# a-rtemis99/hpc_suffix_array

Hardware: AMD Instinct MI355X
Metric: suffixes sorted/sec + ms/doubling-round, 1 GiB input at 1/2/4/8 MI355X (higher is better)
Workload: dtype u32

## Files before the change

### hpc_suffix_array_amd/_native.py

```python
from __future__ import annotations

import ctypes
import os
import subprocess

PKG_DIR = os.path.dirname(os.path.abspath(__file__))
LIB_PATH = os.path.join(PKG_DIR, "lib", "libsa_hip.so")
LIB_PATH = os.environ.get("SA_LIB_PATH", LIB_PATH)
CSRC = os.path.join(PKG_DIR, "csrc")

SA_MAX_ROUNDS = 64
KERNEL_KINDS = ["init", "hist_first", "hist_keys", "scan", "scatter_first", "scatter_keys",
                "heads", "heads_scan", "rerank", "seg_count", "seg_scan", "seg_write", "alphabet", "pack",
                "sort_u", "windows", "local_sort", "pivot_keys", "pivot_count", "pivot_write"]
SCHEDULE_PACKED = 0
SCHEDULE_REFERENCE = 1
ROUND1_AUTO = 0
ROUND1_LSD = 1
ROUND1_BUCKETED = 2
SA_K_COUNT = len(KERNEL_KINDS)
FIND_AUTO = 0
FIND_LANE = 1
FIND_WAVE = 2
FIND_LANE_MAX = 3584
# ... 8 lines not shown
               "sa_count_below_u64_device", "sa_select_u8_device",
               "sa_find_device", "sa_find", "sa_find_ex",
               "sa_match_device", "sa_matching_stats_device", "sa_match", "sa_matching_stats",
               "sa_dist_begin", "sa_dist_cuts", "sa_dist_plan_cuts", "sa_dist_reserve", "sa_dist_release", "sa_dist_round1", "sa_dist_req_count", "sa_dist_req_fill",
               "sa_dist_answer", "sa_dist_refine",
               "sa_last_error", "sa_host_syncs", "sa_device_count", "sa_version", "sa_struct_size"]


class SAError(RuntimeError):
    """A libsa_hip entry point returned an error code."""


DEBUG_FLAGS = {"no_cmp": 0x1, "no_pk8": 0x2, "no_pad": 0x4, "pad_overflow": 0x8, "no_fast32": 0x10,
               "no_pivot": 0x20, "perm_always": 0x40, "no_xq": 0x80, "xq_overflow": 0x100,
               "no_tied": 0x200, "no_key1_round": 0x400, "no_eonly": 0x800,
               "eonly": 0x1000, "fast32_small": 0x2000}


def debug_bits(names) -> int:
    bits = 0
    for x in names or ():
        if x not in DEBUG_FLAGS:
            raise ValueError(f"unknown debug flag {x!r} (one of {sorted(DEBUG_FLAGS)})")
        bits |= DEBUG_FLAGS[x]
    return bits


class SaOpts(ctypes.Structure):
    _fields_ = [("profile", ctypes.c_int32), ("schedule", ctypes.c_int32), ("init_chars", ctypes.c_int32),
                ("radix", ctypes.c_int32), ("round1", ctypes.c_int32), ("debug", ctypes.c_uint32),
                ("span_extra", ctypes.c_int32), ("tune", ctypes.c_int32)]
# ... 217 lines not shown
```

### hpc_suffix_array_amd/csrc/sa_bucket.h

```cpp
#pragma once
#include "sa_kernels.h"

namespace sa {

#ifndef SA_BS_BLOCK
#define SA_BS_BLOCK 512
#endif
constexpr int kBsBlock = SA_BS_BLOCK;
#ifndef SA_BS_ITEMS
#define SA_BS_ITEMS 18
#endif
constexpr int kBsItems = SA_BS_ITEMS;
constexpr int kBsCap = kBsBlock * kBsItems;
constexpr uint32_t kWinStride = 1024;
#ifndef SA_BS_WPC
#define SA_BS_WPC 2
#endif
constexpr uint32_t kBsWpc = SA_BS_WPC;
#ifndef SA_BS_GRID
#define SA_BS_GRID (1u << 22)
#endif
constexpr uint32_t kBsGrid = SA_BS_GRID;
constexpr uint64_t kBucketMinN = 1ull << 20;
constexpr uint32_t kLoBits = 8;
// ... 810 lines not shown
    const uint32_t nlist = words[7];
    const uint32_t lane = lane_id();
    for (uint64_t q = (uint64_t)blockIdx.x * kWaves + wave_id(); q < nlist; q += (uint64_t)gridDim.x * kWaves) {
        const uint32_t j = list[q];
        const uint32_t a = ws[j], o = ou[j], c = ou[j + 1] - o, g0 = og[j];
        for (uint32_t k = lane; k < c; k += kWave) {
            const uint32_t x = so.tmp_idx[a + k];
            u_pos[o + k] = so.tmp_pos[a + k];
            u_idx[o + k] = x;
            u_g[o + k] = so.tmp_g[a + k] + g0;
            if (so.tmp_rank) so.rank[rm.slot(x)] = so.tmp_rank[a + k];
        }
    }
}

constexpr int kPcPer = 16;
constexpr int kPcBlock = kBlock * kPcPer;

__device__ __forceinline__ void popc_load(const uint32_t* __restrict__ bits, uint64_t nw, uint64_t b0,
                                          uint32_t (&c)[kPcPer]) {
    if (b0 + kPcPer <= nw) {
#pragma unroll
        for (int q = 0; q < kPcPer / 4; ++q) {
            const uint4 v = reinterpret_cast<const uint4*>(bits + b0)[q];
            c[4 * q] = (uint32_t)__popc(v.x);
            c[4 * q + 1] = (uint32_t)__popc(v.y);
            c[4 * q + 2] = (uint32_t)__popc(v.z);
            c[4 * q + 3] = (uint32_t)__popc(v.w);
        }
    } else {
// ... 1085 lines not shown
```

### hpc_suffix_array_amd/csrc/sa_build.hip

```cpp
#include <hip/hip_runtime.h>

#include <algorithm>
#include <atomic>
#include <chrono>
#include <cstdarg>
#include <cstdio>
#include <cstdlib>
#include <cstring>
#include <mutex>
#include <string>
#include <thread>
#include <vector>

#include "../../include/sa_hip.h"

#ifndef SA_ALPHA_GRID
#define SA_ALPHA_GRID 2048
#endif

#include "sa_bucket.h"
#include "sa_check.h"
#include "sa_kernels.h"
#include "sa_lcp.h"
#include "sa_limits.h"
// ... 18 lines not shown
}

#define SA_HIP(call)                                                                         \
    do {                                                                                     \
        hipError_t e_ = (call);                                                              \
        if (e_ != hipSuccess)                                                                \
            return set_err(SA_E_HIP, "%s failed: %s (%s:%d)", #call, hipGetErrorString(e_),  \
                           __FILE__, __LINE__);                                              \
    } while (0)

static std::atomic<uint64_t> g_host_syncs{0};
static hipError_t host_sync(hipStream_t s) {
    g_host_syncs.fetch_add(1, std::memory_order_relaxed);
    return hipStreamSynchronize(s);
}
static hipError_t host_memcpy(void* dst, const void* src, size_t bytes, hipMemcpyKind kind) {
    g_host_syncs.fetch_add(1, std::memory_order_relaxed);
    return hipMemcpy(dst, src, bytes, kind);
}

#define SA_TRY(...)                      \
    do {                                 \
        const int rc_ = (__VA_ARGS__);   \
        if (rc_) return rc_;             \
    } while (0)

static bool trace_on() {
    static const bool on = std::getenv("SA_TRACE") != nullptr;
    return on;
}
// ... 1 lines not shown
    do {                                                \
        if (trace_on()) {                               \
            std::fprintf(stderr, "[sa] " __VA_ARGS__);  \
            std::fputc('\n', stderr);                   \
        }                                               \
    } while (0)

#ifndef SA_MAX_CHUNKS
#define SA_MAX_CHUNKS 4096
#endif
constexpr uint32_t kMaxChunks = SA_MAX_CHUNKS;
static_assert(kMaxChunks >= 1 && kMaxChunks <= (1u << 20), "chunk scratch sized for at most 2^20 chunks");
constexpr uint64_t kSparseDiv = 8;
constexpr int kEvPool = 256;
constexpr int kRoundEv = SA_MAX_ROUNDS + 1;

static uint64_t align_up(uint64_t x, uint64_t a) { return (x + a - 1) / a * a; }

static uint32_t bit_width(uint64_t x) {
    uint32_t w = 0;
    while (x) { ++w; x >>= 1; }
    return w;
}

static Chunking plan_chunks(uint64_t n) {
    Chunking ch;
    ch.n = n;
    const uint64_t tiles = (n + kTile - 1) / kTile;
    uint64_t tpc = (tiles + kMaxChunks - 1) / kMaxChunks;
    if (tpc == 0) tpc = 1;
// ... 28 lines not shown
    uint32_t* lsd = nullptr;
    uint32_t* lsdx = nullptr;
    uint32_t* segw = nullptr;
    uint64_t* states = nullptr;
    uint32_t epoch = 0;
    int radix = 0;
    int cus = 256;
    uint32_t* member = nullptr;
    uint32_t* hist = nullptr;
    uint32_t* totals = nullptr;
    uint32_t* counts = nullptr;
    uint32_t* words = nullptr;
    uint32_t* alpha = nullptr;
    uint16_t* code = nullptr;
    uint32_t* host_words = nullptr;
    hipEvent_t ev[sa::kEvPool + sa::kRoundEv];
    int ev_ready = 0;
    sa::DistState* dist = nullptr;
    uint32_t dbg = 0;
    int32_t span_extra = 0;
    int32_t tune = 0;
    bool dna = false;
    bool samples_pending = false;
};

namespace sa {

static uint64_t pad_capacity(uint64_t n) { return n + n / 8 + (1ull << 22); }

static uint64_t pad_elems(uint64_t n) {
    const uint64_t m = align_up(std::max<uint64_t>(n, 1), 64);
// ... 144 lines not shown
        if (!on) return;
        hipEventRecord(c->ev[2 * used + 1], s);
        ++used;
    }
    int nr = 0;
    uint64_t mark_bytes[kRoundEv] = {};
    void round_mark() {
        if (nr < kRoundEv) {
            hipEventRecord(c->ev[kEvPool + nr], s);
            uint64_t b = 0;
            if (st)
                for (int k = 0; k < SA_K_COUNT; ++k) b += st->kern_bytes[k];
            mark_bytes[nr] = b;
        }
        ++nr;
    }
    void round_times() {
        const int last = std::min(nr, kRoundEv) - 1;
        if (!st || last < 1) return;
        hipEventSynchronize(c->ev[kEvPool + last]);
        for (int r = 0; r < last && r < st->rounds; ++r) {
            float ms = 0.f;
            hipEventElapsedTime(&ms, c->ev[kEvPool + r], c->ev[kEvPool + r + 1]);
            st->round_ms[r] = ms;
            st->round_bytes[r] = mark_bytes[r + 1] - mark_bytes[r];
        }
    }
    void flush() {
        if (!on || used == 0) return;
        hipEventSynchronize(c->ev[2 * used - 1]);
// ... 626 lines not shown
    const uint64_t base = (uint64_t)sigma + 1;
    const uint32_t kmax = max_chars(base);
    if (req > 0) return std::min<uint32_t>((uint32_t)req, kmax);
    if (sigma <= 1) return kmax;
    const uint32_t kmin = min_chars(sigma, n);
    const uint32_t P = (key_bits(base, kmin) + 7) / 8;
    uint32_t K = kmin;
    while (K + 1 <= kmax && key_bits(base, K + 1) <= 8 * P) ++K;
    return K;
}

constexpr uint64_t kUsAvg = 4;
#ifndef SA_US_TWO_PHASE
#define SA_US_TWO_PHASE 1
#endif
constexpr int kUsFlagWord = 12;

template <class Pos>
static int segments(sa_context* c, const uint64_t* keys, const uint32_t* idx, const Chunking& ch, Pos pos,
                    bool sparse_ok, bool* sparse_out,
                    uint32_t* sa, int uo, hipStream_t s, Timer& tm, sa_stats* st, uint64_t* D, uint64_t* m,
                    uint64_t* G, uint32_t* rank_arr = nullptr, uint64_t rank_off = 0, RankMap rm = RankMap{},
                    uint64_t set_off = 0, uint32_t g_off = 0, uint32_t* gsn = nullptr) {
    if (!rank_arr) rank_arr = c->rank;
    uint32_t* c_h = c->counts;
    uint32_t* c_u = c->counts + kMaxChunks;
    uint32_t* c_uh = c->counts + 2 * kMaxChunks;
    uint32_t* c_l = c->counts + 3 * kMaxChunks;
    tm.begin(SA_K_SEG_COUNT);
    hipLaunchKernelGGL(k_seg_count, dim3(ch.chunks), dim3(kBlock), 0, s, keys, ch, c_h, c_u, c_uh, c_l);
    tm.end();
// ... 286 lines not shown
    if (bucketed && bp.bs.cmp && short_suffix_ties(h_tail, n, tail_n, h_code, sigma, bp.bs.s, bp.bs.R))
        bucketed = plan_bucketed(sigma, n, Kb, r1, c->radix, &bp, 1, 0);
    const bool force_eonly = (c->dbg & SA_DEBUG_EONLY) != 0;
    if (bucketed && bp.bs.cmp == 1 && ((sigma & (sigma - 1)) != 0 || force_eonly) && !(c->dbg & SA_DEBUG_NO_EONLY)) {
        const uint32_t hb = bp.bs.bb - kLoBits;
        BucketPlan b2;
        if ((force_eonly || !plan_pk8(bp, hb, c->dbg, true)) && plan_bucketed(sigma, n, Kb, r1, c->radix, &b2, 1, 2) &&
            (force_eonly || plan_pk8(b2, hb, c->dbg, true)) &&
            !short_suffix_ties(h_tail, n, tail_n, h_code, sigma, b2.bs.s, b2.bs.R, b2.K))
            bp = b2;
    }
    bool fused = false;
    bool r1_pivot = false;
    uint64_t D = 0, m = 0, G = 0;
    uint64_t seg1[3] = {0, 0, 0};
    if (bucketed) {
        bool done = false;
        rc = round1_bucketed(c, d_text, n, d_sa, bp, full_range(bp, n), s, tm, st, &done, &fused, seg1, &ksh1);
        if (rc) return rc;
        bucketed = done;
        if (done) {
            keys1 = c->keys[0];
            P = 2;
            K = bp.K;
        }
    }
    if (!bucketed) {
        const uint32_t bits1 = key_bits(base, K);
        SA_TRACE("packed: sigma=%u K=%u bits=%u", sigma, K, bits1);
        uint64_t top = 1;
        for (uint32_t t = 1; t < K; ++t) top *= base;
        if (c->radix == 0) {
            rc = onesweep_prepare(c, s);
// ... 43 lines not shown
                        bucketed ? 1u : 0u, bp.bs, bucketed ? c->segw + kBstartOff : nullptr, d_sa, ksh1};
    if (st) st->sparse_ranks = sparse ? 1 : 0;
    auto ensure_samples = [&]() -> int {
        if (!c->samples_pending) return SA_OK;
        c->samples_pending = false;
        const uint64_t ns = (n + (1ull << ksh1) - 1) >> ksh1;
        const uint32_t g = (uint32_t)std::max<uint64_t>(1, std::min<uint64_t>((ns + kBlock - 1) / kBlock, 8192));
        tm.begin(SA_K_SORT_U);
        hipLaunchKernelGGL(k_key1_samples, dim3(g), dim3(kBlock), 0, s, d_text, n, (const uint16_t*)c->code, bp.bs,
                           (const uint32_t*)d_sa, ksh1, keys1);
        tm.end();
        SA_HIP(hipGetLastError());
        add_bytes(st, SA_K_SORT_U, 12 * ns);
        return SA_OK;
    };
    tm.round_mark();
    record_round(st, 0.f, D, P, n, K);
    SA_TRACE("  round 1: D=%llu unsorted=%llu groups=%llu", (unsigned long long)D, (unsigned long long)m,
             (unsigned long long)G);

    const uint32_t wr = bit_width(n);
    for (uint64_t h = K; m > 0; h *= 2) {
        if (h >= 2 * n) return set_err(SA_E_INTERNAL, "doubling did not converge (h=%llu)", (unsigned long long)h);
        const uint32_t wg = G > 1 ? bit_width(G - 1) : 0;
        const uint32_t bits = wg + wr;
        if (bits > 64) return set_err(SA_E_INTERNAL, "key of %u bits", bits);
        const Chunking cu = plan_chunks(m);
        const int ui = uo;
        uo ^= 1;
        uint64_t* sorted = nullptr;
        bool segs_done = false;
        uint64_t Du = 0, m2 = 0, G2 = 0;
        uint32_t kb1 = 0;
        if (bucketed && sparse && h == K && !(c->dbg & SA_DEBUG_NO_KEY1_ROUND)) {
            unsigned __int128 dmax = 1;
            for (uint32_t t = 0; t < bp.bs.s; ++t) dmax *= bp.bs.sigma;
            const unsigned __int128 kmax = ((dmax - 1) << bp.bs.rb) | (((unsigned __int128)1 << bp.bs.rb) - 1);
            uint32_t kw = 0;
            for (unsigned __int128 x = kmax + 1; x; x >>= 1) ++kw;
            kb1 = kw;
        }
        const bool key1_round = kb1 > 0 && kb1 + wg <= 64;
        if (c->radix == 0 && G > 0 && m <= kUsAvg * G) {
            if (sparse && !(SA_US_TWO_PHASE && key1_round)) {
                rc = ensure_samples();
                if (rc) return rc;
            }
            SA_HIP(hipMemsetAsync(c->words + kUsFlagWord, 0, 4, s));
            const uint32_t grid = (uint32_t)std::min<uint64_t>((m + kBlock - 1) / kBlock, 8192);
            tm.begin(SA_K_SORT_U);
#if SA_US_TWO_PHASE
            const uint32_t gk = (uint32_t)std::min<uint64_t>((m + kBlock - 1) / kBlock, 65536);
            if (sparse && key1_round)
                hipLaunchKernelGGL(k_usort_keys<SrcUKey1>, dim3(gk), dim3(kBlock), 0, s,
                                   SrcUKey1{c->u_idx[ui], c->u_g[ui], rl, h, kb1}, m, ukb0);
            else if (sparse)
// ... 543 lines not shown
    if (hipDeviceGetAttribute(&c->cus, hipDeviceAttributeMultiprocessorCount, device) != hipSuccess || c->cus <= 0)
        c->cus = 256;
    if (hipMalloc(&c->hist, (size_t)kRadix * kMaxChunks * 4) != hipSuccess ||
        hipMalloc(&c->totals, kRadix * 4) != hipSuccess || hipMalloc(&c->counts, 4 * kMaxChunks * 4) != hipSuccess ||
        hipMalloc(&c->words, 64) != hipSuccess || hipMalloc(&c->alpha, 256 * 4) != hipSuccess ||
        hipMalloc(&c->code, 256 * 2) != hipSuccess ||
        hipMalloc(&c->os, (2 * kMaxPasses * kRadix + kMaxPasses) * 4) != hipSuccess ||
        hipMalloc(&c->lsd, (2 * kMaxPasses * kLsdMaxRadix + kMaxPasses) * 4 + 64) != hipSuccess ||
        hipMalloc(&c->lsdx, kLsdXqWords * 4) != hipSuccess ||
        hipMalloc(&c->segw, (kBstartOff + 2 * kBstartWords) * 4) != hipSuccess ||
        hipHostMalloc(&c->host_words, 16384, hipHostMallocDefault) != hipSuccess) {
        (void)hipGetLastError();
        sa_context_destroy(c);
        return set_err(SA_E_NOMEM, "context allocation failed");
    }
    for (int i = 0; i < kEvPool + kRoundEv; ++i) {
        if (hipEventCreate(&c->ev[i]) != hipSuccess) {
            sa_context_destroy(c);
            return set_err(SA_E_HIP, "hipEventCreate failed");
        }
        c->ev_ready = i + 1;
    }
    if (max_n) {
        int rc = ensure_capacity(c, max_n);
        if (rc) {
            sa_context_destroy(c);
            return rc;
        }
    }
    *out = c;
    return SA_OK;
// ... 588 lines not shown
```

### hpc_suffix_array_amd/csrc/sa_round1.h

```cpp
#pragma once

#ifndef SA_HIST_WPC
#define SA_HIST_WPC 64
#endif
#ifndef SA_REC_STRIPED
#define SA_REC_STRIPED 1
#endif
#ifndef SA_BB_EXTRA
#define SA_BB_EXTRA 0
#endif
#ifndef SA_ITEMS_A
#define SA_ITEMS_A 12
#endif
#ifndef SA_TEXT_BLOCK
#define SA_TEXT_BLOCK 512
#endif
#ifndef SA_LIST_BLOCK
#define SA_LIST_BLOCK 1024
#endif


#ifndef SA_SEG_BLOCK
#define SA_SEG_BLOCK 1024
#endif
// ... 23 lines not shown
}

static uint32_t text_stripes(const sa_context* c) {
    const uint32_t e = ((uint32_t)c->tune >> 8) & 0xFFu;
    const uint32_t v = e ? e : 8u;
    return v >= 8 ? 8u : v >= 4 ? 4u : v >= 2 ? 2u : 1u;
}

__global__ __launch_bounds__(kLoRadix) void k_sum_rows(const uint32_t* __restrict__ in, uint32_t rows,
                                                       uint32_t* __restrict__ out) {
    uint32_t t = 0;
    for (uint32_t r = 0; r < rows; ++r) t += in[r * kLoRadix + threadIdx.x];
    out[threadIdx.x] = t;
}
constexpr uint64_t kPadMaxN = 1ull << 31;
constexpr uint32_t kPadStartOff = kLoRadix + 1024;
constexpr uint32_t kPadDenseOff = kPadStartOff + kLoRadix + 64;

struct BucketPlan {
    BucketSpec bs{};
    uint32_t ib = 0;
    uint32_t K = 0;
};

static bool plan_bucketed(uint32_t sigma, uint64_t n, uint32_t K, int round1, int radix, BucketPlan* p,
                          int world = 1, int cmp = 0) {
    if (round1 == SA_ROUND1_LSD || radix != 0 || sigma < 2 || n < 2) return false;
    if (round1 == SA_ROUND1_AUTO && n < kBucketMinN) return false;
    uint32_t bb = std::max<uint32_t>(16u, bit_width(n - 1) > 13 ? bit_width(n - 1) - 13 : 0u);
    if (world <= 1) bb = std::min<uint32_t>(bb, 18u);
// ... 92 lines not shown
static BucketRange full_range(const BucketPlan& bp, uint64_t n) {
    BucketRange r;
    r.blo = 0;
    r.bhi = 1u << bp.bs.bb;
    r.m = n;
    return r;
}

static uint32_t range_hb(uint32_t nb) {
    const uint32_t w = bit_width(nb > 1 ? nb - 1 : 1);
    return std::max<uint32_t>(7u, w > kLoBits ? w - kLoBits : 0u);
}

static int round1_bucketed(sa_context* c, const uint8_t* d_text, uint64_t n, uint32_t* d_sa, const BucketPlan& bp,
                           const BucketRange& br_, hipStream_t s, Timer& tm, sa_stats* st, bool* done, bool* fused,
                           uint64_t seg[3], uint32_t* ksh, bool allow_pad = true, bool allow_xq = true) {
    *done = false;
    *fused = false;
    *ksh = 0;
    const uint64_t m = br_.m;
    const uint32_t blo = br_.blo, bhi = br_.bhi;
    if (bhi <= blo || bhi - blo > (1u << 18)) return set_err(SA_E_INTERNAL, "bucket range [%u, %u)", blo, bhi);
    int rc = onesweep_prepare(c, s);
    if (rc) return rc;
    SA_HIP(hipMemsetAsync(c->words, 0, 12, s));
    SA_HIP(hipMemsetAsync(c->words + 5, 0, 28, s));
    const bool listed = m * 10 <= n * 3;
    uint64_t* const lkeys = c->keys_u;
    uint32_t* const lpos = c->vals_u;
    const uint64_t rtiles = (n + kTile - 1) / kTile;
    const uint32_t rgrid = (uint32_t)(std::min<uint64_t>(rtiles, (uint64_t)SA_HIST_WPC * (uint32_t)c->cus) /
                                      kRecStripes * kRecStripes);
    const uint64_t rcap64 = (c->dbg & SA_DEBUG_PAD_OVERFLOW) ? m / kRecStripes / 2 + 1
                                                             : (m + m / 8) / kRecStripes + 2 * (uint64_t)kTile;
// ... 40 lines not shown
        if (striped) {
            SA_HIP(hipMemsetAsync(rcur, 0, kRecStripes * kRecCurStride * 4, s));
            if (ident) SA_HIST_ID_G(rgrid, 3, rcur);
            else if (pow2 && SA_DNA_SWAR && c->dna)
                hipLaunchKernelGGL((k_bucket_hist<true, false, 3, false, true>), dim3(rgrid), dim3(kBlock), 0, s, d_text,
                                   n, (const uint16_t*)c->code, bp.bs, os_ghist(c), 0ull, n, blo, bhi, lkeys, lpos, rcur,
                                   rcap, c->words + 11);
            else if (pow2) SA_HIST_G(rgrid, true, 3, rcur);
            else SA_HIST_G(rgrid, false, 3, rcur);
            SA_HIP(hipMemcpyAsync(c->host_words + 11, c->words + 11, 4, hipMemcpyDeviceToHost, s));
            SA_HIP(host_sync(s));
            if (c->host_words[11]) {
                SA_TRACE("  bucketed round 1: a record stripe overflowed, again with the counting scan");
                tm.end();
                const int rc = round1_bucketed(c, d_text, n, d_sa, bp, br_, s, tm, st, done, fused, seg, ksh, false,
                                               allow_xq);
                if (st) st->round1_segments = 4;
                return rc;
            }
        } else if (ident && listed) SA_HIST_ID(1, wgcnt);
        else if (pow2 && listed) SA_HIST(true, 1, wgcnt);
        else if (pow2) SA_HIST(true, 0, wgcnt);
        else if (listed) SA_HIST(false, 1, wgcnt);
        else SA_HIST(false, 0, wgcnt);
        if (listed && !striped) {
            hipLaunchKernelGGL(k_exscan_u32, dim3(1), dim3(kBlock), 0, s, (const uint32_t*)wgcnt, wgoff, g);
            if (ident) SA_HIST_ID(2, wgoff);
            else if (pow2) SA_HIST(true, 2, wgoff);
            else SA_HIST(false, 2, wgoff);
        }
#undef SA_HIST
// ... 209 lines not shown
    const uint64_t nw = (m + kWinStride - 1) / kWinStride;
    uint32_t* ws = c->vals_alt;
    uint32_t* list = c->vals_alt + nw + 1;
    tm.begin(SA_K_WINDOWS);
    {
        const uint32_t g1 = (uint32_t)std::min<uint64_t>((nw + kBlock) / kBlock, 8192);
        hipLaunchKernelGGL(k_window_starts_tab, dim3(g1), dim3(kBlock), 0, s, (const uint32_t*)(c->segw + kBstartOff),
                           nb_tab, m, nw, ws, list + 4 * nw + 2);
        const uint32_t g2 = (uint32_t)std::min<uint64_t>((nw + kBlock - 1) / kBlock, 1024);
        hipLaunchKernelGGL(k_window_list, dim3(g2), dim3(kBlock), 0, s, (const uint32_t*)ws, nw, list, c->words);
    }
    tm.end();
    add_bytes(st, SA_K_WINDOWS, 8 * nw);
    SA_HIP(hipGetLastError());
    SA_HIP(hipMemcpyAsync(c->host_words, c->words, 48, hipMemcpyDeviceToHost, s));
    SA_HIP(host_sync(s));
    if (c->host_words[4]) return set_err(SA_E_INTERNAL, "radix look-back did not complete");
    if (padded && c->host_words[11]) {
        SA_TRACE("  bucketed round 1: padded segment overflow, again with exact digit totals");
        const int rc = round1_bucketed(c, d_text, n, d_sa, bp, br_, s, tm, st, done, fused, seg, ksh, false, allow_xq);
        if (st) st->round1_segments = 2;
        return rc;
    }
    if (xq && c->host_words[9]) {
        SA_TRACE("  bucketed round 1: second-pass queue overflow, again with one region");
        return round1_bucketed(c, d_text, n, d_sa, bp, br_, s, tm, st, done, fused, seg, ksh, allow_pad, false);
    }
    if (st) st->largest_window = (int32_t)std::min<uint32_t>(c->host_words[5], INT32_MAX);
    if (c->host_words[5] > (uint32_t)kBsCap) {
        SA_TRACE("  bucketed round 1: window of %u > %d suffixes, full sort instead", c->host_words[5], kBsCap);
        return SA_OK;
    }
    uint32_t* skew = list + nw;
    uint32_t* cnt_u = skew + nw;
    uint32_t* cnt_g = cnt_u + nw + 1;
    BucketRel br{cnt_g + nw + 1, c->segw + kBstartOff, c->segw + kBstartOff + kBstartWords, bp.bs.rb};
    br.bits1 = bits1;
    SA_HIP(hipMemsetAsync(cnt_u, 0, (2 * nw + 2) * 4, s));
    uint32_t* const rank_arr = br_.rank ? br_.rank : c->rank;
    uint32_t* const member = br_.member ? br_.member : c->member;
    SA_HIP(hipMemsetAsync(member, 0, (n + 31) / 32 * 4, s));
    SegOut so{rank_arr, member, br_.sa_off, c->u_pos[1], c->u_idx[1], c->u_g[1], cnt_u, cnt_g, kKeySample};
    so.tmp_rank = br_.prefix ? br_.tmp_rank : nullptr;
    so.samples = (SA_LAZY_SAMPLES && !br_.always_u && !(c->dbg & SA_DEBUG_NO_KEY1_ROUND)) ? 0u : 1u;
    uint32_t* const retry = cnt_g + 2 * nw + 2;
    BucketRel br_measured = br;
    br_measured.bits1 = 0;
    uint4* const hdr = reinterpret_cast<uint4*>(((uintptr_t)(retry + nw + 4) + 15) & ~(uintptr_t)15);
    uint32_t* const hx = xq ? reinterpret_cast<uint32_t*>(hdr + nw + 1) : nullptr;
    constexpr uint32_t kBsRows = (kBsBlock / kWave) * kBsItems;
    uint32_t* const xrows = xq ? hx + 16 * (nw + 1) : nullptr;
    const uint64_t* const wide_in = xq ? c->keys[1] : c->keys_u;
    auto local_sort = [&](const SegOut& o) {
        const uint32_t g = std::max<uint32_t>(1, std::min(c->host_words[7], kBsGrid));
        (void)hipMemsetAsync(c->words + kRetryWord, 0, 12, s);
        if (fast32) {
            const uint32_t gs = (uint32_t)std::max<uint64_t>(1, std::min<uint64_t>((nw + kBlock - 1) / kBlock, 1024));
            const bool cr = xq && !(((uint32_t)c->tune >> 29) & 1u);
            hipLaunchKernelGGL(k_window_split, dim3(gs), dim3(kBlock), 0, s, (const uint32_t*)list, (const uint32_t*)ws,
                               br, c->words, hdr, retry, 1u, (const uint32_t*)xq_pc, (const uint32_t*)xq_pn, nb_tab, hx,
                               cr ? kBsRows : 0u);
            if (xq) {
                if (cr)
                    hipLaunchKernelGGL(k_window_rows<true>, dim3(2048), dim3(kBlock), 0, s, (const uint32_t*)c->words,
                                       (const uint4*)hdr, (const uint32_t*)hx, kBsRows, xrows);
                else
                    hipLaunchKernelGGL(k_window_rows<false>, dim3(2048), dim3(kBlock), 0, s, (const uint32_t*)c->words,
                                       (const uint4*)hdr, (const uint32_t*)hx, kBsRows, xrows);
                XqWin xw;
                xw.hx = hx;
// ... 38 lines not shown
        if (br.bits1)
            hipLaunchKernelGGL((k_bucket_sort_wide<kBsBlock, kBsItems>), dim3(std::min<uint32_t>(g, 1024)),
                               dim3(kBsBlock), 0, s, wide_in, br_measured, (const uint32_t*)ws,
                               (const uint32_t*)retry, c->words, bp.ib, c->keys[0], d_sa, skew, o, (uint32_t*)nullptr,
                               (uint32_t)kRetryWord);
        const uint32_t gl = std::min<uint32_t>(g, 1024);
        hipLaunchKernelGGL((k_bucket_sort_lsd<kBsBlock, kBsItems>), dim3(gl), dim3(kBsBlock), 0, s,
                           wide_in, br, (const uint32_t*)ws, (const uint32_t*)skew, c->words, bp.ib,
                           c->keys[0], d_sa, o);
    };
    tm.begin(SA_K_LOCAL_SORT);
    local_sort(so);
    tm.end();
    add_bytes(st, SA_K_LOCAL_SORT, 12 * m + (so.samples ? (m >> kKeySample) * 8 : 0));
    SA_HIP(hipGetLastError());
    tm.begin(SA_K_SEG_WRITE);
    {
        const uint32_t wb = (uint32_t)((nw + 1 + kWsBlock - 1) / kWsBlock);
        uint32_t* part = c->hist;
        hipLaunchKernelGGL(k_wscan_reduce, dim3(wb), dim3(kBlock), 0, s, (const uint32_t*)cnt_u, (const uint32_t*)cnt_g,
                           nw, part);
        hipLaunchKernelGGL(k_wscan_top, dim3(1), dim3(kBlock), 0, s, part, wb);
        hipLaunchKernelGGL(k_wscan_apply, dim3(wb), dim3(kBlock), 0, s, cnt_u, cnt_g, nw, (const uint32_t*)part);
        const uint32_t g = (uint32_t)std::max<uint64_t>(1, std::min<uint64_t>((c->host_words[7] + kWaves - 1) / kWaves, 4096));
        RankMap rm;
        if (br_.prefix) {
            const uint64_t nwb = (n + 31) / 32;
            const uint32_t pb = (uint32_t)((nwb + kPcBlock - 1) / kPcBlock);
            uint32_t* ppart = br_.prefix + nwb + 1;
            hipLaunchKernelGGL(k_popc_reduce, dim3(pb), dim3(kBlock), 0, s, (const uint32_t*)member, nwb, ppart);
            hipLaunchKernelGGL(k_popc_top, dim3(1), dim3(kPcTop), 0, s, ppart, pb);
            hipLaunchKernelGGL(k_popc_apply, dim3(pb), dim3(kBlock), 0, s, (const uint32_t*)member, nwb,
                               (const uint32_t*)ppart, br_.prefix);
            rm = RankMap{member, br_.prefix};
        }
        hipLaunchKernelGGL(k_u_gather, dim3(g), dim3(kBlock), 0, s, (const uint32_t*)list, (const uint32_t*)c->words,
                           (const uint32_t*)ws, (const uint32_t*)cnt_u, (const uint32_t*)cnt_g, so, c->u_pos[0],
                           c->u_idx[0], c->u_g[0], rm);
    }
    tm.end();
    SA_HIP(hipGetLastError());
    SA_HIP(hipMemcpyAsync(c->host_words, c->words, 64, hipMemcpyDeviceToHost, s));
    SA_HIP(host_sync(s));
    if (st) {
        const uint32_t wv[4] = {c->host_words[7], c->host_words[kHdrWord], c->host_words[kRetryWord], c->host_words[10]};
        for (int t = 0; t < 4; ++t) st->round1_windows[t] = (int32_t)std::min<uint32_t>(wv[t], INT32_MAX);
    }
    if (c->host_words[6]) {
        SA_TRACE("  bucketed round 1: local sort flags %u, full sort instead", c->host_words[6]);
        return SA_OK;
    }
    seg[0] = c->host_words[0];
    seg[1] = c->host_words[1];
    seg[2] = c->host_words[2];
    add_bytes(st, SA_K_LOCAL_SORT, seg[1] * 28);
    add_bytes(st, SA_K_SEG_WRITE, 8 * (2 * nw + 2) + seg[1] * 24);
    if (!br_.always_u && seg[1] > n / kSparseDiv) {
        SegOut full{};
        full.ksh = 0;
        SA_HIP(hipMemsetAsync(c->words + 10, 0, 4, s));
        tm.begin(SA_K_LOCAL_SORT);
        local_sort(full);
        tm.end();
        add_bytes(st, SA_K_LOCAL_SORT, 20 * m);
        SA_HIP(hipGetLastError());
    } else {
        *ksh = kKeySample;
        *fused = true;
        c->samples_pending = so.samples == 0u;
    }
    SA_TRACE("  bucketed round 1: s=%u R=%u rb=%u cmp=%u pk8=%d windows=%u (skewed %u) largest=%u", bp.bs.s, bp.bs.R,
             bp.bs.rb, bp.bs.cmp, pk8 ? 1 : 0, c->host_words[7], c->host_words[10], c->host_words[5]);
// ... 4 lines not shown
```

### include/sa_hip.h

```cpp
#ifndef SA_HIP_H
#define SA_HIP_H

#include <stdint.h>

#ifdef __cplusplus
extern "C" {
#endif

#define SA_OK 0
#define SA_E_INVALID (-1)
#define SA_E_NOMEM (-2)
#define SA_E_HIP (-3)
#define SA_E_INTERNAL (-4)

#define SA_MAX_ROUNDS 64

enum sa_kernel_kind {
    SA_K_INIT = 0,
    SA_K_HIST_FIRST = 1,
    SA_K_HIST_KEYS = 2,
    SA_K_SCAN = 3,
    SA_K_SCATTER_FIRST = 4,
    SA_K_SCATTER_KEYS = 5,
    SA_K_HEADS = 6,
// ... 23 lines not shown

#define SA_DEBUG_NO_CMP 0x1u
#define SA_DEBUG_NO_PK8 0x2u
#define SA_DEBUG_NO_PAD 0x4u
#define SA_DEBUG_PAD_OVERFLOW 0x8u
#define SA_DEBUG_NO_FAST32 0x10u
#define SA_DEBUG_NO_PIVOT 0x20u
#define SA_DEBUG_PERM_ALWAYS 0x40u
#define SA_DEBUG_NO_XQ 0x80u
#define SA_DEBUG_XQ_OVERFLOW 0x100u
#define SA_DEBUG_NO_KEY1_ROUND 0x400u
#define SA_DEBUG_NO_TIED 0x200u
#define SA_DEBUG_NO_EONLY 0x800u
#define SA_DEBUG_EONLY 0x1000u
#define SA_DEBUG_FAST32_SMALL 0x2000u

typedef struct {
    int32_t profile;
    int32_t schedule;
    int32_t init_chars;
    int32_t radix;
    int32_t round1;
    uint32_t debug;
    int32_t span_extra;
    int32_t tune;
} sa_opts;

typedef struct {
    int32_t rounds;
    int32_t n_kinds;
// ... 146 lines not shown
```

### profiles/summarize.py

```python
#!/usr/bin/env python3
import csv
import glob
import json
import os
import shutil
import sys
from collections import defaultdict

KINDS = [("k_chk_bin<1024, 8, sa::IsaSrc", "lcp_isa_bin"), ("k_chk_split<1024, 8, 32, 3", "lcp_isa_split"), ("k_perm_split<1024, 8, 32, true, 3", "lcp_isa_split"), ("k_perm_place<1024, false, 3", "lcp_isa_place"), ("k_chk_bin<1024, 8, sa::PlcpSrc", "lcp_place_bin"), ("k_chk_split<1024, 8, 32, 4", "lcp_place_split"), ("k_perm_split<1024, 8, 32, true, 4", "lcp_place_split"), ("k_perm_place<1024, false, 4", "lcp_place_place"), ("k_lcp_best", "lcp_best"), ("k_chk_bin<1024, 8, sa::ChkSrcA", "check_bin_a"), ("k_chk_bin<1024, 8, sa::ChkSrcB", "check_bin_b"),
         ("k_chk_bin<1024, 8, sa::PhiSrc", "lcp_phi_bin"), ("k_chk_split<1024, 8, 32, 2", "lcp_phi_split"),
         ("k_perm_split<1024, 8, 32, true, 2", "lcp_phi_split"), ("k_perm_place<1024, false, 2", "lcp_phi_place"),
         ("k_perm_split<1024, 8, 32, true", "check_split_a"), ("k_perm_split<1024, 8, 40, true", "check_split_b"),
         ("k_chk_split<1024, 8, 32", "check_split_a"), ("k_chk_split<1024, 8, 40", "check_split_b"),
         ("k_perm_place<1024, false, 1", "check_place_a"), ("k_chk_place", "check_place_b"),
         ("k_chk_cursors", "check_small"), ("k_chk_tiles", "check_small"),
         ("k_plcp_irreducible", "lcp_irreducible"), ("k_plcp_long", "lcp_long"),
         ("k_plcp_settle", "lcp_long"), ("k_chunk_max", "lcp_scan"), ("k_scan_chunk_max", "lcp_scan"),
         ("k_plcp_apply", "lcp_scan"), ("k_lcp_gather", "lcp_gather"),
         ("k_pivot_keys", "pivot_keys"), ("k_pivot_pass<0", "pivot_count"), ("k_pivot_pass<1", "pivot_count"), ("k_pivot_pass<2", "pivot_write"),
         ("k_pivot_pass<3", "pivot_write"), ("k_pivot_tied_scan", "pivot_write"),
         ("k_pivot_place", "pivot_place"), ("k_pivot_gp", "pivot_gp"), ("k_lsd_hist", "lsd_hist"),
         ("k_lsd_base", "lsd_base"), ("k_lsd<", "lsd"), ("k_perm_rank", "perm_rank"), ("k_perm_split", "perm_split"),
         ("k_perm_place", "perm_place"), ("k_tile_heads", "heads"), ("k_items_to_sa", "items_to_sa"),
         ("k_split_list", "scatter_first"), ("k_usort_small", "sort_u_small"), ("k_usort_keys", "sort_u_keys"),
         ("k_bucket_sample", "pack"), ("k_window_split", "windows"), ("k_window_list", "windows"),
         ("k_split_text", "scatter_first"), ("k_split_seg", "scatter_keys"), ("k_split<sa::SrcBucketKeys", "scatter_keys"),
         ("k_bucket_hist", "pack"), ("k_bucket_starts", "bucket_starts"),
         ("k_init_rank", "init"), ("k_hist<sa::SrcRank>", "hist_rank"), ("k_hist<sa::SrcText>", "hist_text"),
         ("k_hist<sa::SrcU", "hist_u"), ("k_hist<sa::SrcKeys>", "hist_keys"),
         ("k_scan_rows", "scan"), ("k_scatter<sa::SrcRank>", "scatter_rank"),
         ("k_scatter<sa::SrcText>", "scatter_text"), ("k_scatter<sa::SrcU", "scatter_u"),
         ("k_scatter<sa::SrcKeysIota>", "scatter_iota"), ("k_pack_text", "pack"),
         ("k_scatter<sa::SrcKeys>", "scatter_keys_rs"),
         ("k_onesweep<sa::SrcKeysIota", "scatter_iota"), ("k_onesweep<sa::SrcKeys,", "scatter_keys"),
         ("k_onesweep<sa::SrcBucketIota", "scatter_first"), ("k_onesweep<sa::SrcBucketKeys", "scatter_keys"),
         ("k_pack_bucket", "pack"), ("k_window_starts", "windows"), ("k_window_max", "windows"),
         ("k_bucket_sort_lsd", "local_sort_lsd"), ("k_bucket_sort", "local_sort"),
         ("k_materialize", "sort_u_keys"), ("k_wscan_", "seg_write"), ("k_u_gather", "seg_write"),
         ("k_onesweep<sa::SrcU", "scatter_u"), ("k_onesweep<sa::SrcRank", "scatter_rank"),
# ... 130 lines not shown
```

Measured before the change: 103.6 billion.

## Finish round 2 directly from local-sort staging with a wave-level window sorter

Adds a kernel that, after the bucketed round-1 local sort, sorts each small unsorted group in registers by the next key1 word and scatters the suffixes straight into the SA. This skips the u-gather/compaction and the whole second doubling round when every group fits in a wave and keys are distinct. On any overflow or tie it sets a flag and falls back to the gather path. It also overlaps the member/cnt memsets with the host wait by using an event sync, and merges two small memsets into one.

```diff
diff --git a/hpc_suffix_array_amd/_native.py b/hpc_suffix_array_amd/_native.py
--- a/hpc_suffix_array_amd/_native.py
+++ b/hpc_suffix_array_amd/_native.py
@@ -46,7 +46,7 @@
 DEBUG_FLAGS = {"no_cmp": 0x1, "no_pk8": 0x2, "no_pad": 0x4, "pad_overflow": 0x8, "no_fast32": 0x10,
                "no_pivot": 0x20, "perm_always": 0x40, "no_xq": 0x80, "xq_overflow": 0x100,
                "no_tied": 0x200, "no_key1_round": 0x400, "no_eonly": 0x800,
-               "eonly": 0x1000, "fast32_small": 0x2000}
+               "eonly": 0x1000, "fast32_small": 0x2000, "no_round2_fused": 0x4000}
 
 
 def debug_bits(names) -> int:
diff --git a/hpc_suffix_array_amd/csrc/sa_bucket.h b/hpc_suffix_array_amd/csrc/sa_bucket.h
--- a/hpc_suffix_array_amd/csrc/sa_bucket.h
+++ b/hpc_suffix_array_amd/csrc/sa_bucket.h
@@ -848,6 +848,100 @@
     }
 }
 
+constexpr int kR2Batch = 16;
+
+__global__ __launch_bounds__(kBlock) void k_round2_windows(const uint32_t* __restrict__ list, const uint32_t* words,
+                                                           const uint32_t* __restrict__ ws,
+                                                           const uint32_t* __restrict__ cnt_u,
+                                                           const uint32_t* __restrict__ tmp_pos,
+                                                           const uint32_t* __restrict__ tmp_idx,
+                                                           const uint32_t* __restrict__ tmp_g,
+                                                           const uint8_t* __restrict__ text, uint64_t n,
+                                                           const uint16_t* __restrict__ code, BucketSpec bs, uint64_t m,
+                                                           uint32_t* __restrict__ sa, uint32_t* flag) {
+    const uint32_t nlist = words[7];
+    const uint32_t lane = lane_id();
+    const uint32_t K = bs.s + bs.R;
+    const CodeMap map{code};
+    const uint64_t lt = lanemask_lt(), lem = lt | (1ull << lane);
+    for (uint64_t q0 = ((uint64_t)blockIdx.x * kWaves + wave_id()) * kR2Batch; q0 < nlist;
+         q0 += (uint64_t)gridDim.x * kWaves * kR2Batch) {
+        if (__builtin_amdgcn_readfirstlane((int)__atomic_load_n(flag, __ATOMIC_RELAXED))) return;
+        uint32_t a_l = 0, c_l = 0;
+        if (lane < (uint32_t)kR2Batch && q0 + lane < nlist) {
+            const uint32_t j = list[q0 + lane];
+            c_l = cnt_u[j];
+            a_l = ws[j];
+        }
+        if (__ballot(c_l > (uint32_t)kWave)) {
+            if (lane == 0) atomicOr(flag, 1u);
+            return;
+        }
+        const uint32_t e_l = wave_inclusive_sum(c_l);
+        uint64_t todo = __ballot(c_l != 0);
+        uint32_t base = 0;
+        while (todo) {
+            const uint64_t fit = todo & __ballot(e_l - base <= (uint32_t)kWave);
+            todo &= ~fit;
+            uint32_t a = 0, off = 0, nbase = base;
+            bool act = false;
+            for (uint64_t f = fit; f; f &= f - 1) {
+                const int w = __builtin_ctzll(f);
+                const uint32_t ew = (uint32_t)__shfl((int)e_l, w, kWave), cw = (uint32_t)__shfl((int)c_l, w, kWave);
+                const uint32_t aw = (uint32_t)__shfl((int)a_l, w, kWave);
+                const uint32_t s0 = ew - cw - base;
+                if (lane >= s0 && lane < s0 + cw) {
+                    a = aw;
+                    off = lane - s0;
+                    act = true;
+                }
+                nbase = ew;
+            }
+            base = nbase;
+            bool bad = act && (uint64_t)a + off >= m;
+            act = act && !bad;
+            uint32_t pos = 0, x = 0, g = 0;
+            if (act) {
+                pos = tmp_pos[a + off];
+                x = tmp_idx[a + off];
+                g = tmp_g[a + off];
+            }
+            bad = bad || (act && x >= n);
+            uint64_t key = 0;
+            if (act && !bad && (uint64_t)x + K < n) {
+                uint32_t D;
+                key = key1_words<true>(text, n, map, bs, (uint64_t)x + K, &D) + 1u;
+            }
+            const uint64_t ma = __ballot(act);
+            const uint32_t gp = (uint32_t)__shfl_up((int)g, 1, kWave);
+            const bool head = act && (lane == 0 || off == 0 || g != gp || !((ma >> (lane - 1)) & 1ull));
+            const uint64_t mh = __ballot(head);
+            const uint64_t hl = mh & lem, ab = (mh | ~ma) & ~lem;
+            const uint32_t start = hl ? 63u - (uint32_t)__clzll(hl) : lane;
+            const uint32_t end = ab ? (uint32_t)__builtin_ctzll(ab) : (uint32_t)kWave;
+            const uint32_t len = end - start;
+            bad = bad || (act && len > (uint32_t)kUsLimit);
+            uint32_t rank = 0;
+#pragma unroll
+            for (int t = 0; t < kUsLimit; ++t) {
+                const uint32_t src = (start + t) & (kWave - 1);
+                const uint64_t kk = __shfl(key, (int)src, kWave);
+                if (act && (uint32_t)t < len && src != lane) {
+                    rank += kk < key ? 1u : 0u;
+                    bad = bad || kk == key;
+                }
+            }
+            const uint64_t p = (uint64_t)(uint32_t)__shfl((int)pos, (int)start, kWave) + rank;
+            bad = bad || (act && p >= m);
+            if (__ballot(bad)) {
+                if (lane == 0) atomicOr(flag, 1u);
+                return;
+            }
+            if (act) sa[p] = x;
+        }
+    }
+}
+
 constexpr int kPcPer = 16;
 constexpr int kPcBlock = kBlock * kPcPer;
 
diff --git a/hpc_suffix_array_amd/csrc/sa_build.hip b/hpc_suffix_array_amd/csrc/sa_build.hip
--- a/hpc_suffix_array_amd/csrc/sa_build.hip
+++ b/hpc_suffix_array_amd/csrc/sa_build.hip
@@ -56,6 +56,10 @@
     g_host_syncs.fetch_add(1, std::memory_order_relaxed);
     return hipStreamSynchronize(s);
 }
+static hipError_t host_sync_event(hipEvent_t e) {
+    g_host_syncs.fetch_add(1, std::memory_order_relaxed);
+    return hipEventSynchronize(e);
+}
 static hipError_t host_memcpy(void* dst, const void* src, size_t bytes, hipMemcpyKind kind) {
     g_host_syncs.fetch_add(1, std::memory_order_relaxed);
     return hipMemcpy(dst, src, bytes, kind);
@@ -87,6 +91,7 @@
 constexpr uint64_t kSparseDiv = 8;
 constexpr int kEvPool = 256;
 constexpr int kRoundEv = SA_MAX_ROUNDS + 1;
+constexpr int kSyncEv = kEvPool + kRoundEv;
 
 static uint64_t align_up(uint64_t x, uint64_t a) { return (x + a - 1) / a * a; }
 
@@ -145,7 +150,7 @@
     uint32_t* alpha = nullptr;
     uint16_t* code = nullptr;
     uint32_t* host_words = nullptr;
-    hipEvent_t ev[sa::kEvPool + sa::kRoundEv];
+    hipEvent_t ev[sa::kEvPool + sa::kRoundEv + 1];
     int ev_ready = 0;
     sa::DistState* dist = nullptr;
     uint32_t dbg = 0;
@@ -320,6 +325,9 @@
             mark_bytes[nr] = b;
         }
         ++nr;
+    }
+    void round_unmark() {
+        if (nr > 0) --nr;
     }
     void round_times() {
         const int last = std::min(nr, kRoundEv) - 1;
@@ -976,7 +984,6 @@
 #ifndef SA_US_TWO_PHASE
 #define SA_US_TWO_PHASE 1
 #endif
-constexpr int kUsFlagWord = 12;
 
 template <class Pos>
 static int segments(sa_context* c, const uint64_t* keys, const uint32_t* idx, const Chunking& ch, Pos pos,
@@ -1293,9 +1300,11 @@
     bool r1_pivot = false;
     uint64_t D = 0, m = 0, G = 0;
     uint64_t seg1[3] = {0, 0, 0};
+    int r2 = 0;
     if (bucketed) {
         bool done = false;
-        rc = round1_bucketed(c, d_text, n, d_sa, bp, full_range(bp, n), s, tm, st, &done, &fused, seg1, &ksh1);
+        rc = round1_bucketed(c, d_text, n, d_sa, bp, full_range(bp, n), s, tm, st, &done, &fused, seg1, &ksh1, true,
+                             true, &r2);
         if (rc) return rc;
         bucketed = done;
         if (done) {
@@ -1369,10 +1378,19 @@
         add_bytes(st, SA_K_SORT_U, 12 * ns);
         return SA_OK;
     };
-    tm.round_mark();
+    if (r2 == 0) tm.round_mark();
     record_round(st, 0.f, D, P, n, K);
     SA_TRACE("  round 1: D=%llu unsorted=%llu groups=%llu", (unsigned long long)D, (unsigned long long)m,
              (unsigned long long)G);
+    if (r2 == 2) {
+        tm.round_mark();
+        D = n;
+        record_round(st, 0.f, D, 1, m, 2 * (uint64_t)K);
+        SA_TRACE("  round h=%u: sorted %llu from the local sort's staging, D=%llu", K, (unsigned long long)m,
+                 (unsigned long long)D);
+        m = 0;
+        G = 0;
+    }
 
     const uint32_t wr = bit_width(n);
     for (uint64_t h = K; m > 0; h *= 2) {
@@ -1387,14 +1405,7 @@
         bool segs_done = false;
         uint64_t Du = 0, m2 = 0, G2 = 0;
         uint32_t kb1 = 0;
-        if (bucketed && sparse && h == K && !(c->dbg & SA_DEBUG_NO_KEY1_ROUND)) {
-            unsigned __int128 dmax = 1;
-            for (uint32_t t = 0; t < bp.bs.s; ++t) dmax *= bp.bs.sigma;
-            const unsigned __int128 kmax = ((dmax - 1) << bp.bs.rb) | (((unsigned __int128)1 << bp.bs.rb) - 1);
-            uint32_t kw = 0;
-            for (unsigned __int128 x = kmax + 1; x; x >>= 1) ++kw;
-            kb1 = kw;
-        }
+        if (bucketed && sparse && h == K && !(c->dbg & SA_DEBUG_NO_KEY1_ROUND)) kb1 = key1_bits(bp.bs);
         const bool key1_round = kb1 > 0 && kb1 + wg <= 64;
         if (c->radix == 0 && G > 0 && m <= kUsAvg * G) {
             if (sparse && !(SA_US_TWO_PHASE && key1_round)) {
@@ -1968,7 +1979,7 @@
         sa_context_destroy(c);
         return set_err(SA_E_NOMEM, "context allocation failed");
     }
-    for (int i = 0; i < kEvPool + kRoundEv; ++i) {
+    for (int i = 0; i < kEvPool + kRoundEv + 1; ++i) {
         if (hipEventCreate(&c->ev[i]) != hipSuccess) {
             sa_context_destroy(c);
             return set_err(SA_E_HIP, "hipEventCreate failed");
diff --git a/hpc_suffix_array_amd/csrc/sa_round1.h b/hpc_suffix_array_amd/csrc/sa_round1.h
--- a/hpc_suffix_array_amd/csrc/sa_round1.h
+++ b/hpc_suffix_array_amd/csrc/sa_round1.h
@@ -61,6 +61,16 @@
     out[threadIdx.x] = t;
 }
 constexpr uint64_t kPadMaxN = 1ull << 31;
+constexpr int kUsFlagWord = 12;
+
+static uint32_t key1_bits(const BucketSpec& bs) {
+    unsigned __int128 dmax = 1;
+    for (uint32_t t = 0; t < bs.s; ++t) dmax *= bs.sigma;
+    const unsigned __int128 kmax = ((dmax - 1) << bs.rb) | (((unsigned __int128)1 << bs.rb) - 1);
+    uint32_t kw = 0;
+    for (unsigned __int128 x = kmax + 1; x; x >>= 1) ++kw;
+    return kw;
+}
 constexpr uint32_t kPadStartOff = kLoRadix + 1024;
 constexpr uint32_t kPadDenseOff = kPadStartOff + kLoRadix + 64;
 
@@ -183,10 +193,12 @@
 
 static int round1_bucketed(sa_context* c, const uint8_t* d_text, uint64_t n, uint32_t* d_sa, const BucketPlan& bp,
                            const BucketRange& br_, hipStream_t s, Timer& tm, sa_stats* st, bool* done, bool* fused,
-                           uint64_t seg[3], uint32_t* ksh, bool allow_pad = true, bool allow_xq = true) {
+                           uint64_t seg[3], uint32_t* ksh, bool allow_pad = true, bool allow_xq = true,
+                           int* round2 = nullptr) {
     *done = false;
     *fused = false;
     *ksh = 0;
+    if (round2) *round2 = 0;
     const uint64_t m = br_.m;
     const uint32_t blo = br_.blo, bhi = br_.bhi;
     if (bhi <= blo || bhi - blo > (1u << 18)) return set_err(SA_E_INTERNAL, "bucket range [%u, %u)", blo, bhi);
@@ -257,7 +269,7 @@
                 SA_TRACE("  bucketed round 1: a record stripe overflowed, again with the counting scan");
                 tm.end();
                 const int rc = round1_bucketed(c, d_text, n, d_sa, bp, br_, s, tm, st, done, fused, seg, ksh, false,
-                                               allow_xq);
+                                               allow_xq, round2);
                 if (st) st->round1_segments = 4;
                 return rc;
             }
@@ -497,32 +509,35 @@
     add_bytes(st, SA_K_WINDOWS, 8 * nw);
     SA_HIP(hipGetLastError());
     SA_HIP(hipMemcpyAsync(c->host_words, c->words, 48, hipMemcpyDeviceToHost, s));
-    SA_HIP(host_sync(s));
+    uint32_t* skew = list + nw;
+    uint32_t* cnt_u = skew + nw;
+    uint32_t* cnt_g = cnt_u + nw + 1;
+    uint32_t* const rank_arr = br_.rank ? br_.rank : c->rank;
+    uint32_t* const member = br_.member ? br_.member : c->member;
+    SA_HIP(hipEventRecord(c->ev[kSyncEv], s));
+    SA_HIP(hipMemsetAsync(cnt_u, 0, (2 * nw + 2) * 4, s));
+    SA_HIP(hipMemsetAsync(member, 0, (n + 31) / 32 * 4, s));
+    SA_HIP(host_sync_event(c->ev[kSyncEv]));
     if (c->host_words[4]) return set_err(SA_E_INTERNAL, "radix look-back did not complete");
     if (padded && c->host_words[11]) {
         SA_TRACE("  bucketed round 1: padded segment overflow, again with exact digit totals");
-        const int rc = round1_bucketed(c, d_text, n, d_sa, bp, br_, s, tm, st, done, fused, seg, ksh, false, allow_xq);
+        const int rc = round1_bucketed(c, d_text, n, d_sa, bp, br_, s, tm, st, done, fused, seg, ksh, false, allow_xq,
+                                       round2);
         if (st) st->round1_segments = 2;
         return rc;
     }
     if (xq && c->host_words[9]) {
         SA_TRACE("  bucketed round 1: second-pass queue overflow, again with one region");
-        return round1_bucketed(c, d_text, n, d_sa, bp, br_, s, tm, st, done, fused, seg, ksh, allow_pad, false);
+        return round1_bucketed(c, d_text, n, d_sa, bp, br_, s, tm, st, done, fused, seg, ksh, allow_pad, false,
+                               round2);
     }
     if (st) st->largest_window = (int32_t)std::min<uint32_t>(c->host_words[5], INT32_MAX);
     if (c->host_words[5] > (uint32_t)kBsCap) {
         SA_TRACE("  bucketed round 1: window of %u > %d suffixes, full sort instead", c->host_words[5], kBsCap);
         return SA_OK;
     }
-    uint32_t* skew = list + nw;
-    uint32_t* cnt_u = skew + nw;
-    uint32_t* cnt_g = cnt_u + nw + 1;
     BucketRel br{cnt_g + nw + 1, c->segw + kBstartOff, c->segw + kBstartOff + kBstartWords, bp.bs.rb};
     br.bits1 = bits1;
-    SA_HIP(hipMemsetAsync(cnt_u, 0, (2 * nw + 2) * 4, s));
-    uint32_t* const rank_arr = br_.rank ? br_.rank : c->rank;
-    uint32_t* const member = br_.member ? br_.member : c->member;
-    SA_HIP(hipMemsetAsync(member, 0, (n + 31) / 32 * 4, s));
     SegOut so{rank_arr, member, br_.sa_off, c->u_pos[1], c->u_idx[1], c->u_g[1], cnt_u, cnt_g, kKeySample};
     so.tmp_rank = br_.prefix ? br_.tmp_rank : nullptr;
     so.samples = (SA_LAZY_SAMPLES && !br_.always_u && !(c->dbg & SA_DEBUG_NO_KEY1_ROUND)) ? 0u : 1u;
@@ -536,7 +551,8 @@
     const uint64_t* const wide_in = xq ? c->keys[1] : c->keys_u;
     auto local_sort = [&](const SegOut& o) {
         const uint32_t g = std::max<uint32_t>(1, std::min(c->host_words[7], kBsGrid));
-        (void)hipMemsetAsync(c->words + kRetryWord, 0, 12, s);
+        static_assert(kRetryWord == kUsFlagWord + 1, "one memset clears words[12..15]");
+        (void)hipMemsetAsync(c->words + kUsFlagWord, 0, 16, s);
         if (fast32) {
             const uint32_t gs = (uint32_t)std::max<uint64_t>(1, std::min<uint64_t>((nw + kBlock - 1) / kBlock, 1024));
             const bool cr = xq && !(((uint32_t)c->tune >> 29) & 1u);
@@ -605,8 +621,7 @@
     tm.end();
     add_bytes(st, SA_K_LOCAL_SORT, 12 * m + (so.samples ? (m >> kKeySample) * 8 : 0));
     SA_HIP(hipGetLastError());
-    tm.begin(SA_K_SEG_WRITE);
-    {
+    auto gather_u = [&]() {
         const uint32_t wb = (uint32_t)((nw + 1 + kWsBlock - 1) / kWsBlock);
         uint32_t* part = c->hist;
         hipLaunchKernelGGL(k_wscan_reduce, dim3(wb), dim3(kBlock), 0, s, (const uint32_t*)cnt_u, (const uint32_t*)cnt_g,
@@ -628,8 +643,24 @@
         hipLaunchKernelGGL(k_u_gather, dim3(g), dim3(kBlock), 0, s, (const uint32_t*)list, (const uint32_t*)c->words,
                            (const uint32_t*)ws, (const uint32_t*)cnt_u, (const uint32_t*)cnt_g, so, c->u_pos[0],
                            c->u_idx[0], c->u_g[0], rm);
-    }
-    tm.end();
+    };
+    const bool try_r2 = round2 && so.rank && !br_.always_u && !so.tmp_rank && br_.sa_off == 0 &&
+                        !(c->dbg & (SA_DEBUG_NO_KEY1_ROUND | SA_DEBUG_NO_ROUND2_FUSED)) && key1_bits(bp.bs) <= 64;
+    if (try_r2) {
+        tm.round_mark();
+        tm.begin(SA_K_SORT_U);
+        const uint64_t per = (uint64_t)kWaves * kR2Batch;
+        const uint32_t g = (uint32_t)std::max<uint64_t>(1, std::min<uint64_t>((c->host_words[7] + per - 1) / per, 65536));
+        hipLaunchKernelGGL(k_round2_windows, dim3(g), dim3(kBlock), 0, s, (const uint32_t*)list,
+                           (const uint32_t*)c->words, (const uint32_t*)ws, (const uint32_t*)cnt_u,
+                           (const uint32_t*)so.tmp_pos, (const uint32_t*)so.tmp_idx, (const uint32_t*)so.tmp_g, d_text, n,
+                           (const uint16_t*)c->code, bp.bs, m, d_sa, c->words + kUsFlagWord);
+        tm.end();
+    } else {
+        tm.begin(SA_K_SEG_WRITE);
+        gather_u();
+        tm.end();
+    }
     SA_HIP(hipGetLastError());
     SA_HIP(hipMemcpyAsync(c->host_words, c->words, 64, hipMemcpyDeviceToHost, s));
     SA_HIP(host_sync(s));
@@ -639,14 +670,33 @@
     }
     if (c->host_words[6]) {
         SA_TRACE("  bucketed round 1: local sort flags %u, full sort instead", c->host_words[6]);
+        if (try_r2) tm.round_unmark();
         return SA_OK;
     }
     seg[0] = c->host_words[0];
     seg[1] = c->host_words[1];
     seg[2] = c->host_words[2];
     add_bytes(st, SA_K_LOCAL_SORT, seg[1] * 28);
-    add_bytes(st, SA_K_SEG_WRITE, 8 * (2 * nw + 2) + seg[1] * 24);
-    if (!br_.always_u && seg[1] > n / kSparseDiv) {
+    const bool sparse = br_.always_u || seg[1] <= n / kSparseDiv;
+    if (try_r2) {
+        add_bytes(st, SA_K_SORT_U, seg[1] * 28);
+        if (!sparse) {
+            tm.round_unmark();
+        } else if (c->host_words[kUsFlagWord] == 0) {
+            SA_TRACE("  bucketed round 1: round 2 finished from the staging (%llu members)",
+                     (unsigned long long)seg[1]);
+            *round2 = 2;
+        } else {
+            SA_TRACE("  bucketed round 1: round 2 from the staging gave up, the set compacted");
+            *round2 = 1;
+            tm.begin(SA_K_SEG_WRITE);
+            gather_u();
+            tm.end();
+            SA_HIP(hipGetLastError());
+        }
+    }
+    if (!try_r2 || *round2 == 1) add_bytes(st, SA_K_SEG_WRITE, 8 * (2 * nw + 2) + seg[1] * 24);
+    if (!sparse) {
         SegOut full{};
         full.ksh = 0;
         SA_HIP(hipMemsetAsync(c->words + 10, 0, 4, s));
diff --git a/include/sa_hip.h b/include/sa_hip.h
--- a/include/sa_hip.h
+++ b/include/sa_hip.h
@@ -61,6 +61,7 @@
 #define SA_DEBUG_NO_EONLY 0x800u
 #define SA_DEBUG_EONLY 0x1000u
 #define SA_DEBUG_FAST32_SMALL 0x2000u
+#define SA_DEBUG_NO_ROUND2_FUSED 0x4000u
 
 typedef struct {
     int32_t profile;
diff --git a/profiles/summarize.py b/profiles/summarize.py
--- a/profiles/summarize.py
+++ b/profiles/summarize.py
@@ -22,7 +22,7 @@
          ("k_pivot_place", "pivot_place"), ("k_pivot_gp", "pivot_gp"), ("k_lsd_hist", "lsd_hist"),
          ("k_lsd_base", "lsd_base"), ("k_lsd<", "lsd"), ("k_perm_rank", "perm_rank"), ("k_perm_split", "perm_split"),
          ("k_perm_place", "perm_place"), ("k_tile_heads", "heads"), ("k_items_to_sa", "items_to_sa"),
-         ("k_split_list", "scatter_first"), ("k_usort_small", "sort_u_small"), ("k_usort_keys", "sort_u_keys"),
+         ("k_split_list", "scatter_first"), ("k_round2_windows", "round2_windows"), ("k_usort_small", "sort_u_small"), ("k_usort_keys", "sort_u_keys"),
          ("k_bucket_sample", "pack"), ("k_window_split", "windows"), ("k_window_list", "windows"),
          ("k_split_text", "scatter_first"), ("k_split_seg", "scatter_keys"), ("k_split<sa::SrcBucketKeys", "scatter_keys"),
          ("k_bucket_hist", "pack"), ("k_bucket_starts", "bucket_starts"),
```

New measurement: 105.9 billion, median of 6. +2.2%, better.
